# maxgillett/tinysplat

Measured on AMD Instinct MI355X. Metric: Gaussians*pixels/s fwd+bwd, higher is better.
Workload: dtype f32; 1 GPU; 1000000 random Gaussians, SH degree 3, 1920x1080, fwd+bwd (RGB), BASELINE configs[2]; max_per_tile=614, parallelism=single GPU, tile_lists=16x16 (gsplat's) (auto), gaussian_order=as generated (i.i.d.)

## Files before the change

### include/tinysplat_hip.h

```cpp
#ifndef TINYSPLAT_HIP_H
#define TINYSPLAT_HIP_H

#include <stdint.h>

#ifdef __cplusplus
extern "C" {
#endif

#define TS_ABI_VERSION 8

#define TS_E_BADARG (-1)
#define TS_E_DEGREE (-2)

#define TS_TILE 16
#define TS_SPLAT_RECORD_FLOATS 12
#define TS_PARTIAL_ROW_FLOATS 12

int ts_abi_version(void);

typedef struct ts_camera {
    float fx, fy, cx, cy;
    int32_t img_width, img_height;
    int32_t tile_bounds_x, tile_bounds_y;
    int32_t tile_row0, tile_rows;
    float glob_scale;
    float clip_thresh;
    int32_t wide_tiles;
    int32_t hints;
} ts_camera;
#define TS_HINT_BALANCED_WALK 1
#define TS_HINT_COOP_SPLIT (1 << 20)
#define TS_CAM_LIST_SEGMENTS(s) (((s) & 15) << 8)
#define TS_CAM_WHOLE_TILES(w16) (((w16) & 15) << 12)
#define TS_CAM_COOP_TILES(c16) (((c16) & 15) << 16)
int64_t ts_final_floats(const ts_camera* cam_host, int32_t channels);
int32_t ts_cut_tiles(const ts_camera* cam_host, int32_t* band, int32_t* whole);
int32_t ts_num_tiles(const ts_camera* cam_host);


#define TS_PROJECT_LOG_SCALES 1
#define TS_PROJECT_RAW_QUATS 2

int ts_project_fwd(int32_t n, const float* means3d, const float* scales, const float* quats,
                   const float* viewmat, const float* projmat, const ts_camera* cam_host,
                   int32_t flags, float* xys, float* depths, int32_t* radii, float* conics,
                   int32_t* num_tiles_hit, float* cov3d, void* stream);

int ts_project_bwd(int32_t n, const float* means3d, const float* scales, const float* quats,
                   const float* viewmat, const float* projmat, const ts_camera* cam_host,
                   int32_t flags, const int32_t* radii, const float* v_xy, const float* v_depth,
                   const float* v_conic, const float* v_cov3d,
                   float* v_means3d, float* v_scales, float* v_quats, void* stream);


int ts_sh_fwd(int32_t n, int32_t degrees_to_use, int32_t num_bases, const float* viewdirs,
              const float* coeffs, float* colors, void* stream);

int ts_sh_bwd(int32_t n, int32_t degrees_to_use, int32_t num_bases, const float* viewdirs,
              const float* v_colors, float* v_coeffs, void* stream);

int ts_sh_colors_fwd(int32_t n, int32_t degrees_to_use, int32_t num_bases, const float* means3d,
                     const float* origin, const float* colors_dc, const float* colors_rest,
                     float* colors, uint8_t* clamp_mask, const int32_t* live, void* stream);
int ts_sh_colors_bwd(int32_t n, int32_t degrees_to_use, int32_t num_bases, const float* means3d,
                     const float* origin, const uint8_t* clamp_mask, const float* v_colors,
                     float* v_colors_dc, float* v_colors_rest, void* stream);
int ts_colors_pack_fwd(int32_t n, int32_t degrees_to_use, int32_t num_bases, const float* means3d,
                       const float* origin, const float* colors_dc, const float* colors_rest,
                       uint8_t* clamp_mask, const int32_t* live, int32_t channels, int32_t flags,
                       const float* xys, const int32_t* radii, const float* conics, const float* opacity,
                       const int32_t* cum_tiles_hit, const ts_camera* cam_host, const float* depths,
                       float* splats, void* stream);


int64_t ts_scan_ws_ints(int32_t n);
int ts_scan_tiles(int32_t n, const int32_t* num_tiles_hit, int32_t* cum_tiles_hit,
                  int32_t* scan_ws, int32_t* total_out, void* stream);

int64_t ts_bin_ws_ints(int32_t n, int32_t num_tiles);

int ts_bin_count(int32_t n, const float* xys, const int32_t* radii, const float* splats,
                 const ts_camera* cam_host, int32_t* bin_ws, void* stream);

int ts_tile_offsets(int32_t n, int32_t num_tiles, int32_t* bin_ws, int32_t* tile_bins,
                    const int32_t* cum_tiles_hit, int64_t capacity, void* stream);
int ts_tile_offsets_stats(int32_t n, int32_t num_tiles, int32_t* bin_ws, int32_t* tile_bins,
                          const int32_t* cum_tiles_hit, int64_t capacity, int32_t* longest_list, void* stream);

int ts_bin_scatter(int32_t n, const float* xys, const int32_t* radii, const float* splats,
                   const ts_camera* cam_host, const int32_t* bin_ws, int32_t* bucket_ids, int32_t* scratch,
                   void* stream);

int ts_sort_tiles(int32_t num_tiles, const int32_t* tile_bins, const float* depths,
                  const int32_t* bucket_ids, int32_t* gaussian_ids_sorted, int32_t* sort_ws,
                  int32_t* zeroed_counter, void* stream);
int ts_sort_tiles_above(int32_t num_tiles, const int32_t* tile_bins, const float* depths,
                        const int32_t* bucket_ids, int32_t* gaussian_ids_sorted, int32_t* sort_ws,
                        int32_t* zeroed_counter, void* stream);

int32_t ts_bin_group_form(int32_t n);
int ts_bin_count_groups(int32_t n, const float* xys, const int32_t* radii, const float* splats,
                        const ts_camera* cam_host, int32_t* bin_ws, void* stream);
int ts_group_offsets(int32_t n, int32_t num_tiles, int32_t* bin_ws, int32_t* tile_bins,
                     const int32_t* cum_tiles_hit, int64_t capacity, int32_t* longest_list, void* stream);
int ts_bin_scatter_groups(int32_t n, const float* xys, const int32_t* radii, const float* splats,
                          const ts_camera* cam_host, int32_t* bin_ws, int32_t* tile_bins, int32_t* bucket_ids,
                          int32_t* scratch, void* stream);
int32_t ts_bin_one_walk_form(int32_t n, int32_t num_tiles);
int32_t ts_bin_stage_capacity(void);
int ts_bin_emit_groups(int32_t n, const float* xys, const int32_t* radii, const float* splats,
                       const ts_camera* cam_host, const int32_t* cum_tiles_hit, int64_t capacity, int32_t* bin_ws,
                       int32_t* scratch, void* stream);
int ts_emit_offsets(int32_t n, int32_t num_tiles, int32_t* bin_ws, int32_t* tile_bins,
                    const int32_t* cum_tiles_hit, int64_t capacity, int32_t* longest_list, void* stream);
int ts_bin_gather_groups(int32_t n, int32_t num_tiles, int32_t* bin_ws, int32_t* tile_bins, int32_t* bucket_ids,
                         const int32_t* scratch, void* stream);
int ts_sort_tiles_stats(int32_t num_tiles, const int32_t* tile_bins, const float* depths,
                        const int32_t* bucket_ids, int32_t* gaussian_ids_sorted, int32_t* sort_ws,
                        int32_t* zeroed_counter, int32_t n, const int32_t* bin_ws, int32_t* longest_list,
                        void* stream);
int ts_sort_tiles_above_stats(int32_t num_tiles, const int32_t* tile_bins, const float* depths,
                              const int32_t* bucket_ids, int32_t* gaussian_ids_sorted, int32_t n,
                              const int32_t* bin_ws, int32_t* longest_list, void* stream);

#define TS_RASTER_LOGIT_OPACITY 1

int ts_pack_splats(int32_t n, int32_t channels, int32_t flags, const float* xys, const int32_t* radii,
                   const float* conics, const float* colors, const float* opacity,
                   const int32_t* cum_tiles_hit, const ts_camera* cam_host, const float* depths,
                   float* splats, void* stream);
// ... 375 lines not shown
```

### tinysplat_amd/_lib.py

```python
from __future__ import annotations

import ctypes
import os
from ctypes import POINTER, c_double, c_float, c_int32, c_int64, c_void_p
from pathlib import Path

LIB_PATH = Path(os.environ["TS_LIB_PATH"]) if os.environ.get("TS_LIB_PATH") else \
    Path(__file__).resolve().parent / "csrc" / "libtinysplat_hip.so"
ABI_VERSION = 8
HINT_BALANCED_WALK = 1
HINT_COOP_SPLIT = 1 << 20
RASTER_LOGIT_OPACITY = 1
RASTER_CLAMP_RGB = 2
RASTER_SPLIT_BLOCKS = 4
RASTER_NARROW_WAVES = 8
FRAME_TIGHT = 1
FRAME_SPLIT = 2
FRAME_NARROW_WAVES = 8
FRAME_STRIPE = 16
FRAME_DIRECT_SCATTER = 32
FRAME_PLANES = 64
FRAME_SEPARATE_SORT = 128
FRAME_LIST_STATS = 256
FRAME_SURVIVORS = 512
# ... 30 lines not shown
                    "view34", "projview", "origin", "background",
                    "xys", "depths", "conics", "colors", "splats",
                    "radii", "num_tiles_hit", "cum_tiles_hit", "sh_mask",
                    "scan_ws", "bin_ws", "tile_bins", "total_host")]
                + [("num_intersects", c_int64), ("capacity", c_int64)]
                + [(name, c_void_p) for name in (
                    "bucket_ids", "gaussian_ids_sorted", "out_img", "final_Ts", "final_index", "clamp_mask",
                    "v_out_img", "partials", "row_flags",
                    "v_xy", "v_conic", "v_colors", "v_depth", "v_opacity",
                    "v_means", "v_scales", "v_quats", "v_colors_dc", "v_colors_rest",
                    "out_depth", "v_out_depth", "survivors")])


_FRAME = POINTER(TsFrame)


class TsAdam(ctypes.Structure):
    _fields_ = [("exp_avg", c_void_p * 6), ("exp_avg_sq", c_void_p * 6), ("lr", c_float * 6), ("step", c_int32 * 6),
                ("beta1", c_float), ("beta2", c_float), ("eps", c_float)]


_ADAM = POINTER(TsAdam)

MAX_RANKS = 16


class TsStripes(ctypes.Structure):
    _fields_ = [("num", c_int32), ("row", c_int32 * (MAX_RANKS + 1))]


_STRIPES = POINTER(TsStripes)


class TsRankStep(ctypes.Structure):
    _fields_ = [("stripes", TsStripes), ("group_base", c_int32 * (MAX_RANKS + 1)), ("gid_base", c_int32),
                ("send_rows", c_int32), ("recv_rows", c_int32), ("route_ws", c_void_p), ("counts", c_void_p),
                ("send", c_void_p), ("recv", c_void_p), ("grad_rows", c_void_p), ("back", c_void_p)]


_RANK = POINTER(TsRankStep)

ENTRY_PROBE = ctypes.CFUNCTYPE(None, ctypes.c_char_p, c_int32, c_void_p)

SIGNATURES = {
    "ts_abi_version": (c_int32, []),
    "ts_project_fwd": (c_int32, [c_int32, _P, _P, _P, _P, _P, _CAM, c_int32, _P, _P, _P, _P, _P, _P, _P]),
    "ts_project_bwd": (c_int32, [c_int32, _P, _P, _P, _P, _P, _CAM, c_int32, _P, _P, _P, _P, _P, _P, _P, _P, _P]),
    "ts_sh_fwd": (c_int32, [c_int32, c_int32, c_int32, _P, _P, _P, _P]),
    "ts_sh_bwd": (c_int32, [c_int32, c_int32, c_int32, _P, _P, _P, _P]),
    "ts_sh_colors_fwd": (c_int32, [c_int32, c_int32, c_int32, _P, _P, _P, _P, _P, _P, _P, _P]),
    "ts_sh_colors_bwd": (c_int32, [c_int32, c_int32, c_int32, _P, _P, _P, _P, _P, _P, _P]),
    "ts_scan_ws_ints": (c_int64, [c_int32]),
    "ts_scan_tiles": (c_int32, [c_int32, _P, _P, _P, _P, _P]),
    "ts_bin_ws_ints": (c_int64, [c_int32, c_int32]),
    "ts_bin_count": (c_int32, [c_int32, _P, _P, _P, _CAM, _P, _P]),
    "ts_tile_offsets": (c_int32, [c_int32, c_int32, _P, _P, _P, c_int64, _P]),
    "ts_tile_offsets_stats": (c_int32, [c_int32, c_int32, _P, _P, _P, c_int64, _P, _P]),
    "ts_bin_scatter": (c_int32, [c_int32, _P, _P, _P, _CAM, _P, _P, _P, _P]),
    "ts_sort_tiles": (c_int32, [c_int32, _P, _P, _P, _P, _P, _P, _P]),
    "ts_sort_tiles_above": (c_int32, [c_int32, _P, _P, _P, _P, _P, _P, _P]),
    "ts_bin_group_form": (c_int32, [c_int32]),
    "ts_bin_count_groups": (c_int32, [c_int32, _P, _P, _P, _CAM, _P, _P]),
    "ts_group_offsets": (c_int32, [c_int32, c_int32, _P, _P, _P, c_int64, _P, _P]),
    "ts_bin_scatter_groups": (c_int32, [c_int32, _P, _P, _P, _CAM, _P, _P, _P, _P, _P]),
    "ts_bin_one_walk_form": (c_int32, [c_int32, c_int32]),
    "ts_bin_stage_capacity": (c_int32, []),
    "ts_bin_emit_groups": (c_int32, [c_int32, _P, _P, _P, _CAM, _P, c_int64, _P, _P, _P]),
    "ts_emit_offsets": (c_int32, [c_int32, c_int32, _P, _P, _P, c_int64, _P, _P]),
    "ts_bin_gather_groups": (c_int32, [c_int32, c_int32, _P, _P, _P, _P, _P]),
    "ts_sort_tiles_stats": (c_int32, [c_int32, _P, _P, _P, _P, _P, _P, c_int32, _P, _P, _P]),
    "ts_sort_tiles_above_stats": (c_int32, [c_int32, _P, _P, _P, _P, c_int32, _P, _P, _P]),
    "ts_num_tiles": (c_int32, [_CAM]),
    "ts_final_floats": (c_int64, [_CAM, c_int32]),
    "ts_cut_tiles": (c_int32, [_CAM, _P, _P]),
    "ts_colors_pack_fwd": (c_int32, [c_int32, c_int32, c_int32, _P, _P, _P, _P, _P, _P, c_int32, c_int32,
                                     _P, _P, _P, _P, _P, _CAM, _P, _P, _P]),
    "ts_pack_splats": (c_int32, [c_int32, c_int32, c_int32, _P, _P, _P, _P, _P, _P, _CAM, _P, _P, _P]),
    "ts_raster_fwd": (c_int32, [c_int32, c_int32, _CAM, _P, _P, _P, _P, _P, _P, _P, _P, _P]),
    "ts_raster_bwd": (c_int32, [c_int32, c_int32, c_int64, _CAM, _P, _P, _P, _P, _P, _P, _P, _P, _P, _P, _P, _P]),
    "ts_raster_fwd_planes": (c_int32, [c_int32, c_int32, _CAM, _P, _P, _P, _P, _P, _P, _P, _P, _P, _P]),
    "ts_raster_fwd_sort": (c_int32, [c_int32, c_int32, _CAM, _P, _P, _P, _P, _P, _P, _P, _P, _P, _P, _P, _P]),
    "ts_raster_bwd_planes": (c_int32, [c_int32, c_int32, c_int64, _CAM, _P, _P, _P, _P, _P, _P, _P, _P, c_int32,
                                       _P, _P, _P, _P, _P]),
    "ts_bench_stream_read": (c_int32, [_P, c_int64, _P, _P]),
    "ts_bench_gather48": (c_int32, [_P, _P, c_int64, _P, _P]),
    "ts_photometric_ws_floats": (c_int64, [c_int32, c_int32]),
    "ts_photometric_loss": (c_int32, [c_int32, c_int32, _P, _P, c_float, c_float, _P, _P, _P]),
    "ts_photometric_loss_rgbd": (c_int32, [c_int32, c_int32, c_int32, _P, _P, _P, c_float, c_float, c_float, _P, _P, _P]),
    "ts_photometric_loss_planes": (c_int32, [c_int32, c_int32, _P, _P, _P, _P, c_float, c_float, c_float, _P, _P, _P,
                                             _P]),
    "ts_photometric_loss_reduce": (c_int32, [c_int32, c_int32, c_float, c_float, c_float, _P, _P, _P]),
    "ts_adam_step": (c_int32, [c_int32, _P, _P, _P, _P, _P, _P, _P, c_float, c_float, c_float, _P]),
    "ts_sh_colors_bwd_adam": (c_int32, [c_int32, c_int32, c_int32, _P, _P, _P, _P, _P, _P, _ADAM, _P]),
    "ts_project_bwd_adam": (c_int32, [c_int32, _P, _P, _P, _P, _P, _CAM, c_int32, _P, _P, _P, _P, _P, _P, _ADAM, _P]),
    "ts_frame_bwd_params_adam": (c_int32, [_FRAME, _ADAM, _P]),
    "ts_grad_accum": (c_int32, [c_int32, _P, _P, _P]),
    "ts_densify_classify": (c_int32, [c_int32, _P, _P, _P, POINTER(TsDensifyPolicy), _P, _P]),
    "ts_densify_ws_ints": (c_int64, [c_int32]),
    "ts_densify_plan": (c_int32, [c_int32, _P, _P, _P, _P, _P]),
    "ts_gather_rows": (c_int32, [c_int32, _P, _P, _P, c_int32, c_int32, _P, _P]),
    "ts_split_fixup": (c_int32, [c_int32, _P, _P, _P, _P, _P, _P, _P, _P]),
    "ts_ply_row_floats": (c_int32, [c_int32]),
    "ts_ply_pack_rows": (c_int32, [c_int32, c_int32, _P, _P, _P, _P, _P, _P, _P, _P]),
    "ts_ply_unpack_rows": (c_int32, [c_int32, c_int32, _P, _P, _P, _P, _P, _P, _P, _P]),
    "ts_reduce_partials": (c_int32, [c_int32, c_int32, c_int32, _P, _P, _P, _P, _P, _P, _P, _P, _P, _P, _P, _P]),
    "ts_route_ws_ints": (c_int64, [c_int32, c_int32]),
# ... 134 lines not shown
```

### tinysplat_amd/csrc/binning.hip

```cpp
#include <hip/hip_runtime.h>

#include "../../include/tinysplat_hip.h"
#include "host_util.h"
#include "pack.h"
#include "splat_math.h"

namespace {

constexpr int kThreads = 256;
constexpr int kScanItems = 4;
constexpr int kScanBlock = kThreads * kScanItems;

__device__ __forceinline__ int wave_inclusive_scan(int v) {
    const int lane = threadIdx.x & 63;
#pragma unroll
    for (int d = 1; d < 64; d <<= 1) {
        const int u = __shfl_up(v, d, 64);
        if (lane >= d) v += u;
    }
    return v;
}

template <int WAVES = 4>
__device__ __forceinline__ int block_inclusive_scan(int v, int* total) {
    __shared__ int wave_sums[WAVES];
    const int lane = threadIdx.x & 63, wave = threadIdx.x >> 6;
    int inc = wave_inclusive_scan(v);
    if (lane == 63) wave_sums[wave] = inc;
    __syncthreads();
    int add = 0, tot = 0;
#pragma unroll
    for (int w = 0; w < WAVES; ++w) {
        const int s = wave_sums[w];
        if (w < wave) add += s;
        tot += s;
    }
    *total = tot;
    __syncthreads();
    return inc + add;
}

__global__ __launch_bounds__(kThreads) void scan_local_kernel(int n, const int* __restrict__ in,
                                                              int* __restrict__ out,
                                                              int* __restrict__ block_sums,
                                                              int* __restrict__ total_out) {
    const int base = blockIdx.x * kScanBlock + threadIdx.x * kScanItems;
    int v[kScanItems];
    int sum = 0;
#pragma unroll
    for (int k = 0; k < kScanItems; ++k) {
        v[k] = (base + k < n) ? in[base + k] : 0;
        sum += v[k];
        v[k] = sum;
    }
    int total;
    const int inc = block_inclusive_scan(sum, &total);
    const int excl = inc - sum;
#pragma unroll
    for (int k = 0; k < kScanItems; ++k)
        if (base + k < n) {
            out[base + k] = v[k] + excl;
            if (total_out && gridDim.x == 1 && base + k == n - 1)
                __hip_atomic_store(total_out, v[k] + excl, __ATOMIC_RELEASE, __HIP_MEMORY_SCOPE_SYSTEM);
        }
    if (threadIdx.x == 0) block_sums[blockIdx.x] = total;
}

__global__ __launch_bounds__(kThreads) void scan_add_kernel(int n, int* __restrict__ out,
                                                            const int* __restrict__ block_sums,
                                                            int* __restrict__ total_out) {
    __shared__ int red[kThreads / 64];
    int part = 0;
    for (int j = threadIdx.x; j < (int)blockIdx.x; j += kThreads) part += block_sums[j];
#pragma unroll
    for (int d = 32; d >= 1; d >>= 1) part += __shfl_xor(part, d, 64);
    if ((threadIdx.x & 63) == 0) red[threadIdx.x >> 6] = part;
    __syncthreads();
    int add = 0;
#pragma unroll
    for (int w = 0; w < kThreads / 64; ++w) add += red[w];
    const int base = blockIdx.x * kScanBlock + threadIdx.x * kScanItems;
#pragma unroll
    for (int k = 0; k < kScanItems; ++k)
        if (base + k < n) {
            const int v = out[base + k] + add;
            if (blockIdx.x != 0) out[base + k] = v;
            if (total_out && base + k == n - 1)
                __hip_atomic_store(total_out, v, __ATOMIC_RELEASE, __HIP_MEMORY_SCOPE_SYSTEM);
        }
}

#ifndef TS_BIN_THREADS
#define TS_BIN_THREADS 1024
#endif
constexpr int kBinThreads = TS_BIN_THREADS;
#ifndef TS_BIN_CHUNK
#define TS_BIN_CHUNK 4096
#endif
constexpr int kBinChunkMin = TS_BIN_CHUNK;
constexpr int kBinMaxChunks = 512;
constexpr int kBinWindowMax = 36864;
constexpr int kBinTargetBlocks = 1;

__host__ __device__ inline int bin_num_chunks(int n) {
    int per = n / 192;
    per = per < 1024 ? 1024 : (per > kBinChunkMin ? kBinChunkMin : per);
    int b = (n + per - 1) / per;
    if (b < 1) b = 1;
    if (b > kBinMaxChunks) b = kBinMaxChunks;
    return b;
}

inline int bin_window_tiles(int n, int num_tiles) {
    const int chunks = bin_num_chunks(n);
    int nwin = (kBinTargetBlocks + chunks - 1) / chunks;
    const int max_win = (num_tiles + 255) / 256;
    if (nwin > max_win) nwin = max_win;
    if (nwin < 1) nwin = 1;
    int window = (num_tiles + nwin - 1) / nwin;
    window = (window + 63) & ~63;
    if (window > kBinWindowMax) window = kBinWindowMax;
    return window;
}

using ts::TightTest;

#ifndef TS_BIN_PRE
#define TS_BIN_PRE 2
#endif
constexpr int kBinPre = TS_BIN_PRE;
template <typename Emit>
__device__ __forceinline__ void walk_chunk(int g0, int g1, const float* __restrict__ xys,
                                           const int* __restrict__ radii,
                                           const float4* __restrict__ splats, const ts_camera& cam,
                                           Emit emit) {
    const int ws = cam.wide_tiles ? 1 : 0;
    const int tbx = (cam.tile_bounds_x + ws) >> ws;
    const bool tight_lists = splats != nullptr;
    for (int base = g0 + threadIdx.x; base < g1; base += kBinPre * kBinThreads) {
        int r[kBinPre];
        float2 xy[kBinPre];
        float4 q0[kBinPre], q1[kBinPre];
// ... 1031 lines not shown
    const int* __restrict__ tile_bins, const float* __restrict__ depths,
    const int* __restrict__ bucket_ids, int* __restrict__ ids_sorted,
    const int* __restrict__ large_count, const int* __restrict__ large_list) {
    __shared__ unsigned long long lds_large[kLargeLdsU64];
    const int count = *large_count;
    for (int q = blockIdx.x; q < count; q += gridDim.x) {
        const int2 range = reinterpret_cast<const int2*>(tile_bins)[large_list[q]];
        const int n = range.y - range.x;
        if (n <= kSortCap) continue;
        __syncthreads();
        sort_tile_sample(bucket_ids + range.x, depths, ids_sorted + range.x, n, lds_large);
    }
}

__global__ __launch_bounds__(kThreads) void sort_tiles_above_kernel(
    const int* __restrict__ tile_bins, const float* __restrict__ depths,
    const int* __restrict__ bucket_ids, int* __restrict__ ids_sorted, const ListStats stats) {
    __shared__ unsigned long long lds_u64[kLargeLdsU64 > kSortCap / 2 ? kLargeLdsU64 : kSortCap / 2];
    if (stats.group_max && blockIdx.x == 0) store_longest(stats);
    const int2 range = reinterpret_cast<const int2*>(tile_bins)[blockIdx.x];
    const int n = range.y - range.x;
    if (n <= kWaveSortMax) return;
    if (n <= kSortCap) sort_bucket_block(bucket_ids + range.x, depths, ids_sorted + range.x, n, lds_u64);
    else sort_tile_sample(bucket_ids + range.x, depths, ids_sorted + range.x, n, lds_u64);
}

__global__ __launch_bounds__(kThreads) void pack_splats_kernel(int n, const ts::PackArgs a,
                                                              const float* __restrict__ colors) {
    const int i = blockIdx.x * kThreads + threadIdx.x;
    if (i >= n) return;
    if (a.radii[i] <= 0) return;
    float c0, c1, c2, c3 = 0.0f;
    if (a.channels == 4 && a.depths == nullptr) {
        const float4 c = reinterpret_cast<const float4*>(colors)[i];
        c0 = c.x; c1 = c.y; c2 = c.z; c3 = c.w;
    } else {
        c0 = colors[3 * i]; c1 = colors[3 * i + 1]; c2 = colors[3 * i + 2];
        if (a.channels == 4) c3 = a.depths[i];
    }
    ts::pack_one(a, i, c0, c1, c2, c3);
}

}

extern "C" {

int32_t ts_num_tiles(const ts_camera* cam) {
    if (!cam) return 0;
    const int tbx = cam->wide_tiles ? (cam->tile_bounds_x + 1) / 2 : cam->tile_bounds_x;
    return cam->tile_rows * tbx;
}

int64_t ts_scan_ws_ints(int32_t n) {
    return n <= 0 ? 1 : (int64_t)((n + kScanBlock - 1) / kScanBlock);
}

int ts_scan_tiles(int32_t n, const int32_t* num_tiles_hit, int32_t* cum_tiles_hit,
                  int32_t* scan_ws, int32_t* total_out, void* stream) {
    if (n < 0) return TS_E_BADARG;
    if (n == 0) return 0;
    if (!num_tiles_hit || !cum_tiles_hit || !scan_ws) return TS_E_BADARG;
    hipStream_t s = (hipStream_t)stream;
    const int nb = (n + kScanBlock - 1) / kScanBlock;
    hipLaunchKernelGGL(scan_local_kernel, dim3(nb), dim3(kThreads), 0, s, n, num_tiles_hit,
                       cum_tiles_hit, scan_ws, total_out);
    if (nb > 1)
        hipLaunchKernelGGL(scan_add_kernel, dim3(nb), dim3(kThreads), 0, s, n, cum_tiles_hit, scan_ws,
                           total_out);
    return launch_status();
}

int64_t ts_bin_ws_ints(int32_t n, int32_t num_tiles) { return bin_geometry(n, num_tiles).spare + 1; }

int ts_bin_count(int32_t n, const float* xys, const int32_t* radii, const float* splats,
                 const ts_camera* cam, int32_t* bin_ws, void* stream) {
    if (n < 0 || !cam || !bin_ws) return TS_E_BADARG;
    const int nt = ts_num_tiles(cam);
    if (nt <= 0) return 0;
    if (n > 0 && (!xys || !radii)) return TS_E_BADARG;
    const BinGeometry g = bin_geometry(n, nt);
    const int window = bin_window_tiles(n, nt);
    const int windows = (nt + window - 1) / window;
    const size_t lds = (size_t)window * sizeof(int);
    if (lds > 64 * 1024)
        (void)hipFuncSetAttribute(reinterpret_cast<const void*>(&bin_count_kernel),
                                  hipFuncAttributeMaxDynamicSharedMemorySize, (int)lds);
    hipLaunchKernelGGL(bin_count_kernel, dim3(g.chunks, windows), dim3(kBinThreads), lds,
                       (hipStream_t)stream, n, g.chunk, xys, radii,
                       reinterpret_cast<const float4*>(splats), *cam, nt, window, bin_ws);
    return launch_status();
}

int ts_tile_offsets(int32_t n, int32_t num_tiles, int32_t* bin_ws, int32_t* tile_bins,
                    const int32_t* cum_tiles_hit, int64_t capacity, void* stream) {
    return ts_tile_offsets_stats(n, num_tiles, bin_ws, tile_bins, cum_tiles_hit, capacity, nullptr, stream);
}

int ts_tile_offsets_stats(int32_t n, int32_t num_tiles, int32_t* bin_ws, int32_t* tile_bins,
                          const int32_t* cum_tiles_hit, int64_t capacity, int32_t* longest_list, void* stream) {
    if (n < 0 || num_tiles < 0) return TS_E_BADARG;
    if (num_tiles == 0) return 0;
    if (!bin_ws || !tile_bins) return TS_E_BADARG;
    const BinGeometry g = bin_geometry(n, num_tiles);
    int* tile_total = bin_ws + g.tile_start;
    const int per_group = (g.chunks + kScanGroups - 1) / kScanGroups;
    hipStream_t s = (hipStream_t)stream;
    hipLaunchKernelGGL(column_scan_kernel, dim3((num_tiles + kColTiles - 1) / kColTiles),
                       dim3(kColTiles * kScanGroups), 0, s, num_tiles, g.chunks, per_group, bin_ws, tile_total, true);
    hipLaunchKernelGGL(tile_offsets_kernel, dim3(1), dim3(kOffsetsThreads), 0, s, num_tiles, tile_total,
                       tile_bins, bin_ws + g.spare,
                       (cum_tiles_hit && n > 0) ? cum_tiles_hit + (n - 1) : nullptr, (long long)capacity, longest_list);
    return launch_status();
}

int32_t ts_bin_group_form(int32_t n) { return two_hop(n) ? 1 : 0; }

int ts_bin_count_groups(int32_t n, const float* xys, const int32_t* radii, const float* splats,
                        const ts_camera* cam, int32_t* bin_ws, void* stream) {
    if (!cam || !bin_ws || !xys || !radii || !two_hop(n)) return TS_E_BADARG;
    const int nt = ts_num_tiles(cam);
    if (nt <= 0) return 0;
// ... 221 lines not shown
```

### tinysplat_amd/csrc/frame.hip

```cpp
#include <hip/hip_runtime.h>

#include <atomic>
#include <cstdlib>
#if !defined(TS_NO_ROCTX) && __has_include(<rocprofiler-sdk-roctx/roctx.h>)
#include <rocprofiler-sdk-roctx/roctx.h>
#define TS_HAVE_ROCTX 1
#else
#define TS_HAVE_ROCTX 0
#endif

#include "../../include/tinysplat_hip.h"
#include "raster_survivors.h"

struct TsRange {
#if TS_HAVE_ROCTX
    explicit TsRange(const char* name) { roctxRangePush(name); }
    ~TsRange() { roctxRangePop(); }
#else
    explicit TsRange(const char*) {}
#endif
};

static std::atomic<ts_entry_probe> g_probe{nullptr};
static std::atomic<void*> g_probe_user{nullptr};
// ... 47 lines not shown
    return ((f->cam.hints >> 8) & 15) > 1 && !f->cam.wide_tiles && !(f->flags & TS_FRAME_NARROW_WAVES);
}
inline int bwd_split(const ts_frame* f) {
    return ((f->flags & TS_FRAME_SPLIT) && !segmented(f)) ? TS_RASTER_SPLIT_BLOCKS : 0;
}
inline int small_n_fused() {
    static const int v = [] {
        const char* e = getenv("TS_SMALL_N_FUSED");
        return e ? atoi(e) : 262144;
    }();
    return v;
}
inline bool survivors(const ts_frame* f) {
    return (f->flags & TS_FRAME_SURVIVORS) && f->survivors && f->final_Ts && f->num_intersects > 0 &&
           f->cam.wide_tiles == 0 &&
           !(f->flags & (TS_FRAME_SPLIT | TS_FRAME_NARROW_WAVES | TS_FRAME_SEPARATE_SORT));
}
enum class ListForm { direct, matrix, group, one_walk };
inline ListForm list_form(const ts_frame* f) {
    if ((f->flags & TS_FRAME_DIRECT_SCATTER) || !ts_bin_group_form(f->n)) return ListForm::direct;
    if (!(f->flags & TS_FRAME_GROUP_COUNTS)) return ListForm::matrix;
    if ((f->flags & TS_FRAME_ONE_WALK) && !(f->cam.hints & TS_HINT_BALANCED_WALK) &&
        ts_bin_one_walk_form(f->n, num_tiles(f)))
        return ListForm::one_walk;
    return ListForm::group;
}
inline const float* tight_records(const ts_frame* f) { return (f->flags & TS_FRAME_TIGHT) ? f->splats : nullptr; }
inline int32_t* longest_word(const ts_frame* f) {
    if ((f->flags & TS_FRAME_LIST_STATS) && f->total_host) {
        int32_t* dev = mapped_pointer(f->total_host);
        if (dev) return dev + 1;
    }
    return nullptr;
}
inline int raster_flags(const ts_frame* f) {
    return TS_RASTER_CLAMP_RGB | ((f->flags & TS_FRAME_SPLIT) ? TS_RASTER_SPLIT_BLOCKS : 0) |
           ((f->flags & TS_FRAME_NARROW_WAVES) ? TS_RASTER_NARROW_WAVES : 0);
}
}

extern "C" {

int32_t ts_frame_struct_bytes(void) { return (int32_t)sizeof(ts_frame); }

int ts_set_entry_probe(ts_entry_probe fn, void* user) {
    g_probe_user.store(user, std::memory_order_relaxed);
    g_probe.store(fn, std::memory_order_release);
    return 0;
}

int ts_frame_fwd_project(const ts_frame* f, void* stream) {
    TsRange range_("ts_frame_fwd_project");
    if (bad(f)) return TS_E_BADARG;
    TS_TRY(TS_ENTRY("ts_project_fwd",
                    ts_project_fwd(f->n, f->means, f->scales, f->quats, f->view34, f->projview, &f->cam, 3, f->xys,
                                   f->depths, f->radii, f->conics, f->num_tiles_hit, nullptr, stream)));
    int32_t* total_dev = f->total_host ? mapped_pointer(f->total_host) : nullptr;
    TS_TRY(TS_ENTRY("ts_scan_tiles",
                    ts_scan_tiles(f->n, f->num_tiles_hit, f->cum_tiles_hit, f->scan_ws, total_dev, stream)));
    if (f->n > 0 && f->total_host && !total_dev) {
        const hipError_t e = hipMemcpyAsync(f->total_host, f->cum_tiles_hit + (f->n - 1), sizeof(int32_t),
                                            hipMemcpyDeviceToHost, (hipStream_t)stream);
        if (e != hipSuccess) return (int)e;
    }
    return 0;
}

int ts_frame_fwd_prepare(const ts_frame* f, void* stream) {
    TsRange range_("ts_frame_fwd_prepare");
    if (bad(f)) return TS_E_BADARG;
    TS_TRY(TS_ENTRY("ts_colors_pack_fwd",
                    ts_colors_pack_fwd(f->n, f->sh_degree, f->num_bases, f->means, f->origin, f->colors_dc,
                                       f->num_bases > 1 ? f->colors_rest : nullptr, f->sh_mask,
                                       (f->flags & TS_FRAME_STRIPE) ? f->num_tiles_hit : nullptr, f->channels,
                                       TS_RASTER_LOGIT_OPACITY, f->xys, f->radii, f->conics, f->opacities,
                                       f->cum_tiles_hit, &f->cam, f->channels == 4 ? f->depths : nullptr, f->splats,
                                       stream)));
    const float* tight = tight_records(f);
    switch (list_form(f)) {
    case ListForm::one_walk:
        return 0;
    case ListForm::group:
        TS_TRY(TS_ENTRY("ts_bin_count",
                        ts_bin_count_groups(f->n, f->xys, f->radii, tight, &f->cam, f->bin_ws, stream)));
        return TS_ENTRY("ts_tile_offsets",
                        ts_group_offsets(f->n, num_tiles(f), f->bin_ws, f->tile_bins, f->cum_tiles_hit, f->capacity,
                                         longest_word(f), stream));
    case ListForm::matrix:
    case ListForm::direct:
        TS_TRY(TS_ENTRY("ts_bin_count", ts_bin_count(f->n, f->xys, f->radii, tight, &f->cam, f->bin_ws, stream)));
        return TS_ENTRY("ts_tile_offsets",
                        ts_tile_offsets_stats(f->n, num_tiles(f), f->bin_ws, f->tile_bins, f->cum_tiles_hit,
                                              f->capacity, longest_word(f), stream));
    }
    return TS_E_BADARG;
}

int ts_frame_fwd_composite(const ts_frame* f, void* stream) {
    TsRange range_("ts_frame_fwd_composite");
    if (bad(f) || f->num_intersects < 0) return TS_E_BADARG;
    const bool planes = (f->flags & TS_FRAME_PLANES) != 0;
    if (planes && (f->channels != 4 || !f->out_depth)) return TS_E_BADARG;
    const bool fused_sort = f->num_intersects > 0 && f->cam.wide_tiles == 0 &&
                            !(f->flags & (TS_FRAME_NARROW_WAVES | TS_FRAME_SEPARATE_SORT));
    const ListForm form = list_form(f);
    const float* tight = tight_records(f);
    const bool listed = f->num_intersects > 0;
    int32_t* scratch = f->gaussian_ids_sorted;
    switch (form) {
    case ListForm::one_walk:
        TS_TRY(TS_ENTRY("ts_bin_scatter",
                        ts_bin_emit_groups(f->n, f->xys, f->radii, tight, &f->cam, f->cum_tiles_hit, f->capacity,
// ... 235 lines not shown
```

### tinysplat_amd/csrc/project.hip

```cpp
#include <hip/hip_runtime.h>

#include "../../include/tinysplat_hip.h"
#include "host_util.h"
#include "pack.h"
#include "splat_math.h"
#include "adam_math.h"

namespace {

constexpr int kThreads = 256;
#ifndef TS_SH_THREADS_FWD
#define TS_SH_THREADS_FWD 128
#endif
#ifndef TS_SH_THREADS_BWD
#define TS_SH_THREADS_BWD 256
#endif
typedef float f4v __attribute__((ext_vector_type(4)));
__device__ __forceinline__ void store4(float4* p, float a, float b, float c, float d) {
    f4v v = {a, b, c, d};
    __builtin_nontemporal_store(v, reinterpret_cast<f4v*>(p));
}
constexpr int kShThreadsFwd = TS_SH_THREADS_FWD, kShThreadsBwd = TS_SH_THREADS_BWD;
__device__ __forceinline__ float4 load4_stream(const float4* p) {
    const f4v v = __builtin_nontemporal_load(reinterpret_cast<const f4v*>(p));
    return make_float4(v.x, v.y, v.z, v.w);
}

#include "project_inputs.h"

__global__ __launch_bounds__(kThreads) void project_fwd_kernel(
    int n, const float* __restrict__ means3d, const float* __restrict__ scales,
    const float* __restrict__ quats, const float* __restrict__ viewmat,
    const float* __restrict__ projmat, const ts_camera cam, const int flags,
    float* __restrict__ xys, float* __restrict__ depths, int* __restrict__ radii,
    float* __restrict__ conics, int* __restrict__ num_tiles_hit, float* __restrict__ cov3d) {
    const int i = blockIdx.x * kThreads + threadIdx.x;
    if (i >= n) return;
    const ts::Cam C = load_cam(viewmat, projmat, cam);
    const float m[3] = {means3d[3 * i], means3d[3 * i + 1], means3d[3 * i + 2]};
    float s[3] = {scales[3 * i], scales[3 * i + 1], scales[3 * i + 2]};
    const float4 qv = reinterpret_cast<const float4*>(quats)[i];
    float q[4] = {qv.x, qv.y, qv.z, qv.w};
    prep_inputs(flags, s, q, nullptr);
    ts::ProjOut o;
    ts::project_one(C, m, s, q, o);
    reinterpret_cast<float2*>(xys)[i] = make_float2(o.x, o.y);
    depths[i] = o.depth;
    radii[i] = o.radius;
    conics[3 * i] = o.conic[0]; conics[3 * i + 1] = o.conic[1]; conics[3 * i + 2] = o.conic[2];
    num_tiles_hit[i] = o.tiles;
    if (cov3d) {
        float2* c3 = reinterpret_cast<float2*>(cov3d) + 3 * (size_t)i;
        c3[0] = make_float2(o.cov3d[0], o.cov3d[1]);
        c3[1] = make_float2(o.cov3d[2], o.cov3d[3]);
        c3[2] = make_float2(o.cov3d[4], o.cov3d[5]);
    }
}

struct ProjAdam {
    float *means, *scales, *quats, *opacities;
    const float* v_opacity;
    float *m_means, *v_means, *m_scales, *v_scales, *m_quats, *v_quats, *m_opac, *v_opac;
    ts::AdamCoef c_means, c_scales, c_quats, c_opac;
};
template <bool ADAM>
__global__ __launch_bounds__(kThreads) void project_bwd_kernel(
    int n, const float* __restrict__ means3d, const float* __restrict__ scales,
    const float* __restrict__ quats, const float* __restrict__ viewmat,
    const float* __restrict__ projmat, const ts_camera cam, const int flags,
    const int* __restrict__ radii, const float* __restrict__ v_xy, const float* __restrict__ v_depth,
    const float* __restrict__ v_conic, const float* __restrict__ v_cov3d,
    float* __restrict__ v_means3d, float* __restrict__ v_scales, float* __restrict__ v_quats, const ProjAdam ad) {
    const int i = blockIdx.x * kThreads + threadIdx.x;
    if (i >= n) return;
    ts::ProjGrad g;
    for (int k = 0; k < 3; ++k) { g.v_mean[k] = 0.0f; g.v_scale[k] = 0.0f; }
    for (int k = 0; k < 4; ++k) g.v_quat[k] = 0.0f;
    float pm[3] = {0.f, 0.f, 0.f}, ps[3] = {0.f, 0.f, 0.f}, pq[4] = {0.f, 0.f, 0.f, 0.f};
    if (ADAM) {
        pm[0] = means3d[3 * i]; pm[1] = means3d[3 * i + 1]; pm[2] = means3d[3 * i + 2];
        ps[0] = scales[3 * i]; ps[1] = scales[3 * i + 1]; ps[2] = scales[3 * i + 2];
        const float4 qv = reinterpret_cast<const float4*>(quats)[i];
        pq[0] = qv.x; pq[1] = qv.y; pq[2] = qv.z; pq[3] = qv.w;
    }
    if (radii[i] > 0) {
        const ts::Cam C = load_cam(viewmat, projmat, cam);
        const float m[3] = {ADAM ? pm[0] : means3d[3 * i], ADAM ? pm[1] : means3d[3 * i + 1], ADAM ? pm[2] : means3d[3 * i + 2]};
        float s[3] = {ADAM ? ps[0] : scales[3 * i], ADAM ? ps[1] : scales[3 * i + 1], ADAM ? ps[2] : scales[3 * i + 2]};
        float4 qv;
        if (ADAM) qv = make_float4(pq[0], pq[1], pq[2], pq[3]);
        else qv = reinterpret_cast<const float4*>(quats)[i];
        float q[4] = {qv.x, qv.y, qv.z, qv.w};
        float inv_n = 1.0f;
        prep_inputs(flags, s, q, &inv_n);
        const float2 vxy = reinterpret_cast<const float2*>(v_xy)[i];
        const float vx[2] = {vxy.x, vxy.y};
        const float vc[3] = {v_conic[3 * i], v_conic[3 * i + 1], v_conic[3 * i + 2]};
        float vcov[6];
        if (v_cov3d) {
            for (int k = 0; k < 6; ++k) vcov[k] = v_cov3d[6 * (size_t)i + k];
        }
        ts::project_one_vjp(C, m, s, q, vx, v_depth ? v_depth[i] : 0.0f, vc, v_cov3d ? vcov : nullptr, g);
        if (flags & TS_PROJECT_LOG_SCALES) {
            g.v_scale[0] *= s[0]; g.v_scale[1] *= s[1]; g.v_scale[2] *= s[2];
        }
        if (flags & TS_PROJECT_RAW_QUATS) {
            const float dotp = q[0] * g.v_quat[0] + q[1] * g.v_quat[1] + q[2] * g.v_quat[2] +
                               q[3] * g.v_quat[3];
            for (int k = 0; k < 4; ++k) g.v_quat[k] = (g.v_quat[k] - q[k] * dotp) * inv_n;
// ... 310 lines not shown
#pragma unroll
    for (int u = 0; u < U; ++u) acc[u] = make_float4(0.f, 0.f, 0.f, 0.f);
    for (; i + (U - 1) * stride < n16; i += U * stride) {
        float4 v[U];
#pragma unroll
        for (int u = 0; u < U; ++u) {
            const f4v t = __builtin_nontemporal_load(reinterpret_cast<const f4v*>(src + i + u * stride));
            v[u] = make_float4(t.x, t.y, t.z, t.w);
        }
#pragma unroll
        for (int u = 0; u < U; ++u) {
            acc[u].x += v[u].x; acc[u].y += v[u].y; acc[u].z += v[u].z; acc[u].w += v[u].w;
        }
    }
    for (; i < n16; i += stride) {
        const float4 v0 = src[i];
        acc[0].x += v0.x; acc[0].y += v0.y; acc[0].z += v0.z; acc[0].w += v0.w;
    }
    float t = 0.f;
#pragma unroll
    for (int u = 0; u < U; ++u) t += (acc[u].x + acc[u].y) + (acc[u].z + acc[u].w);
    if (t == 123456.789f) sink[0] = t;
}

__global__ __launch_bounds__(kThreads) void gather48_kernel(const float4* __restrict__ records,
                                                            const int* __restrict__ ids, size_t m,
                                                            float* __restrict__ sink) {
    const size_t stride = (size_t)gridDim.x * kThreads;
    float4 a = make_float4(0.f, 0.f, 0.f, 0.f);
    for (size_t j = (size_t)blockIdx.x * kThreads + threadIdx.x; j < m; j += stride) {
        const size_t g = (size_t)ids[j];
        const float4 q0 = records[3 * g], q1 = records[3 * g + 1], q2 = records[3 * g + 2];
        a.x += q0.x + q1.x + q2.x; a.y += q0.y + q1.y + q2.y; a.z += q0.z + q1.z + q2.z; a.w += q0.w + q1.w + q2.w;
    }
    if ((a.x + a.y) + (a.z + a.w) == 123456.789f) sink[0] = a.x;
}

}

extern "C" {

int ts_abi_version(void) { return TS_ABI_VERSION; }

int ts_project_fwd(int32_t n, const float* means3d, const float* scales, const float* quats,
                   const float* viewmat, const float* projmat, const ts_camera* cam,
                   int32_t flags, float* xys, float* depths, int32_t* radii, float* conics,
                   int32_t* num_tiles_hit, float* cov3d, void* stream) {
    if (n < 0 || !cam) return TS_E_BADARG;
    if (n == 0) return 0;
    if (!means3d || !scales || !quats || !viewmat || !projmat || !xys || !depths || !radii ||
        !conics || !num_tiles_hit)
        return TS_E_BADARG;
    const int grid = (n + kThreads - 1) / kThreads;
    hipLaunchKernelGGL(project_fwd_kernel, dim3(grid), dim3(kThreads), 0, (hipStream_t)stream, n,
                       means3d, scales, quats, viewmat, projmat, *cam, (int)flags, xys, depths, radii,
                       conics, num_tiles_hit, cov3d);
    return launch_status();
}

int ts_project_bwd(int32_t n, const float* means3d, const float* scales, const float* quats,
                   const float* viewmat, const float* projmat, const ts_camera* cam,
                   int32_t flags, const int32_t* radii, const float* v_xy, const float* v_depth,
                   const float* v_conic, const float* v_cov3d, float* v_means3d, float* v_scales,
                   float* v_quats, void* stream) {
    if (n < 0 || !cam) return TS_E_BADARG;
    if (n == 0) return 0;
    if (!means3d || !scales || !quats || !viewmat || !projmat || !radii || !v_xy ||
        !v_conic || !v_means3d || !v_scales || !v_quats)
        return TS_E_BADARG;
    const int grid = (n + kThreads - 1) / kThreads;
    hipLaunchKernelGGL(project_bwd_kernel<false>, dim3(grid), dim3(kThreads), 0, (hipStream_t)stream, n,
                       means3d, scales, quats, viewmat, projmat, *cam, (int)flags, radii, v_xy, v_depth,
                       v_conic, v_cov3d, v_means3d, v_scales, v_quats, ProjAdam{});
    return launch_status();
}

static bool adam_group_ok(const ts_adam* a, int k) {
    return a->exp_avg[k] && a->exp_avg_sq[k] && a->step[k] >= 1;
}

int ts_project_bwd_adam(int32_t n, float* means3d, float* scales, float* quats, const float* viewmat,
                        const float* projmat, const ts_camera* cam, int32_t flags, const int32_t* radii,
                        const float* v_xy, const float* v_depth, const float* v_conic, float* opacities,
                        const float* v_opacity, const ts_adam* adam, void* stream) {
    if (n < 0 || !cam || !adam) return TS_E_BADARG;
    if (n == 0) return 0;
    if (!means3d || !scales || !quats || !viewmat || !projmat || !radii || !v_xy || !v_conic) return TS_E_BADARG;
    if (!adam_group_ok(adam, TS_ADAM_MEANS) || !adam_group_ok(adam, TS_ADAM_SCALES) || !adam_group_ok(adam, TS_ADAM_QUATS))
        return TS_E_BADARG;
    if (opacities && (!v_opacity || !adam_group_ok(adam, TS_ADAM_OPACITIES))) return TS_E_BADARG;
    ProjAdam ad{};
    ad.means = means3d; ad.scales = scales; ad.quats = quats; ad.opacities = opacities; ad.v_opacity = v_opacity;
    ad.m_means = adam->exp_avg[TS_ADAM_MEANS]; ad.v_means = adam->exp_avg_sq[TS_ADAM_MEANS];
    ad.m_scales = adam->exp_avg[TS_ADAM_SCALES]; ad.v_scales = adam->exp_avg_sq[TS_ADAM_SCALES];
    ad.m_quats = adam->exp_avg[TS_ADAM_QUATS]; ad.v_quats = adam->exp_avg_sq[TS_ADAM_QUATS];
    ad.m_opac = adam->exp_avg[TS_ADAM_OPACITIES]; ad.v_opac = adam->exp_avg_sq[TS_ADAM_OPACITIES];
    auto coef = [&](int k) { return ts::adam_coef(adam->lr[k], adam->step[k], adam->beta1, adam->beta2, adam->eps); };
    ad.c_means = coef(TS_ADAM_MEANS); ad.c_scales = coef(TS_ADAM_SCALES); ad.c_quats = coef(TS_ADAM_QUATS);
    if (opacities) ad.c_opac = coef(TS_ADAM_OPACITIES);
    const int grid = (n + kThreads - 1) / kThreads;
    hipLaunchKernelGGL(project_bwd_kernel<true>, dim3(grid), dim3(kThreads), 0, (hipStream_t)stream, n,
                       means3d, scales, quats, viewmat, projmat, *cam, (int)flags, radii, v_xy, v_depth,
                       v_conic, (const float*)nullptr, (float*)nullptr, (float*)nullptr, (float*)nullptr, ad);
    return launch_status();
}

static int sh_check(int32_t n, int32_t degree, int32_t num_bases) {
    if (n < 0) return TS_E_BADARG;
    if (num_bases != 1 && num_bases != 4 && num_bases != 9 && num_bases != 16 && num_bases != 25)
// ... 218 lines not shown
```

Before: 2070000 billion Gaussians*pixels/s.

## Fuse tile-count block scan into projection kernel and add a blocked scan-add pass

The projection forward kernel now also runs a per-workgroup inclusive scan of tiles hit and writes local prefix sums plus one block sum per workgroup. A new add kernel then reduces the preceding block sums and adds the offsets with vectorised int4 accesses. This replaces the separate scan-local pass over num_tiles_hit, removing one kernel launch and one read of the counts array. The cost is a larger block-sum workspace, because scan blocks shrink to 256, and a redundant prefix reduction of block sums inside every add block.

After: 2074000 billion Gaussians*pixels/s (median of 2 runs). Within noise of the previous version (+0.2%).

```diff
diff --git a/include/tinysplat_hip.h b/include/tinysplat_hip.h
--- a/include/tinysplat_hip.h
+++ b/include/tinysplat_hip.h
@@ -76,6 +76,11 @@
 int64_t ts_scan_ws_ints(int32_t n);
 int ts_scan_tiles(int32_t n, const int32_t* num_tiles_hit, int32_t* cum_tiles_hit,
                   int32_t* scan_ws, int32_t* total_out, void* stream);
+int ts_project_fwd_scan(int32_t n, const float* means3d, const float* scales, const float* quats,
+                        const float* viewmat, const float* projmat, const ts_camera* cam_host, int32_t flags,
+                        float* xys, float* depths, int32_t* radii, float* conics, int32_t* num_tiles_hit,
+                        float* cov3d, int32_t* cum_tiles_hit, int32_t* scan_ws, int32_t* total_out, void* stream);
+int ts_scan_tiles_add(int32_t n, int32_t* cum_tiles_hit, const int32_t* scan_ws, int32_t* total_out, void* stream);
 
 int64_t ts_bin_ws_ints(int32_t n, int32_t num_tiles);
 
diff --git a/tinysplat_amd/_lib.py b/tinysplat_amd/_lib.py
--- a/tinysplat_amd/_lib.py
+++ b/tinysplat_amd/_lib.py
@@ -106,6 +106,8 @@
     "ts_sh_colors_bwd": (c_int32, [c_int32, c_int32, c_int32, _P, _P, _P, _P, _P, _P, _P]),
     "ts_scan_ws_ints": (c_int64, [c_int32]),
     "ts_scan_tiles": (c_int32, [c_int32, _P, _P, _P, _P, _P]),
+    "ts_project_fwd_scan": (c_int32, [c_int32, _P, _P, _P, _P, _P, _CAM, c_int32, _P, _P, _P, _P, _P, _P, _P, _P, _P, _P]),
+    "ts_scan_tiles_add": (c_int32, [c_int32, _P, _P, _P, _P]),
     "ts_bin_ws_ints": (c_int64, [c_int32, c_int32]),
     "ts_bin_count": (c_int32, [c_int32, _P, _P, _P, _CAM, _P, _P]),
     "ts_tile_offsets": (c_int32, [c_int32, c_int32, _P, _P, _P, c_int64, _P]),
diff --git a/tinysplat_amd/csrc/binning.hip b/tinysplat_amd/csrc/binning.hip
--- a/tinysplat_amd/csrc/binning.hip
+++ b/tinysplat_amd/csrc/binning.hip
@@ -11,34 +11,7 @@
 constexpr int kScanItems = 4;
 constexpr int kScanBlock = kThreads * kScanItems;
 
-__device__ __forceinline__ int wave_inclusive_scan(int v) {
-    const int lane = threadIdx.x & 63;
-#pragma unroll
-    for (int d = 1; d < 64; d <<= 1) {
-        const int u = __shfl_up(v, d, 64);
-        if (lane >= d) v += u;
-    }
-    return v;
-}
-
-template <int WAVES = 4>
-__device__ __forceinline__ int block_inclusive_scan(int v, int* total) {
-    __shared__ int wave_sums[WAVES];
-    const int lane = threadIdx.x & 63, wave = threadIdx.x >> 6;
-    int inc = wave_inclusive_scan(v);
-    if (lane == 63) wave_sums[wave] = inc;
-    __syncthreads();
-    int add = 0, tot = 0;
-#pragma unroll
-    for (int w = 0; w < WAVES; ++w) {
-        const int s = wave_sums[w];
-        if (w < wave) add += s;
-        tot += s;
-    }
-    *total = tot;
-    __syncthreads();
-    return inc + add;
-}
+#include "block_scan.h"
 
 __global__ __launch_bounds__(kThreads) void scan_local_kernel(int n, const int* __restrict__ in,
                                                               int* __restrict__ out,
@@ -88,6 +61,81 @@
             if (total_out && base + k == n - 1)
                 __hip_atomic_store(total_out, v, __ATOMIC_RELEASE, __HIP_MEMORY_SCOPE_SYSTEM);
         }
+}
+
+constexpr int kAddSums = 16;
+constexpr int kAddRounds = kAddSums * kProjectScanBlock / kScanBlock;
+static_assert(kProjectScanBlock == 256 && kThreads / 64 * kProjectScanBlock == kScanBlock, "a wave of a round = one block");
+__global__ __launch_bounds__(kThreads) void scan_add_kernel_proj(int n, int* __restrict__ out,
+                                                                 const int* __restrict__ block_sums,
+                                                                 int* __restrict__ total_out) {
+    __shared__ int red[kThreads / 64];
+    __shared__ int own[kAddSums];
+    const int first = blockIdx.x * kAddSums;
+    const bool vec = (reinterpret_cast<uintptr_t>(out) & 15) == 0;
+    const int base0 = blockIdx.x * (kAddSums * kProjectScanBlock) + threadIdx.x * kScanItems;
+    int4 v[kAddRounds];
+#pragma unroll
+    for (int r = 0; r < kAddRounds; ++r) {
+        const int base = base0 + r * kScanBlock;
+        if (vec && base + kScanItems <= n) v[r] = *reinterpret_cast<const int4*>(out + base);
+    }
+    int part = 0;
+    if ((reinterpret_cast<uintptr_t>(block_sums) & 15) == 0) {
+        const int4* sums4 = reinterpret_cast<const int4*>(block_sums);
+        for (int j0 = 0; j0 < first / 4; j0 += 4 * kThreads) {
+            int4 q[4];
+#pragma unroll
+            for (int u = 0; u < 4; ++u) {
+                const int j = j0 + u * kThreads + threadIdx.x;
+                q[u] = j < first / 4 ? sums4[j] : make_int4(0, 0, 0, 0);
+            }
+#pragma unroll
+            for (int u = 0; u < 4; ++u) part += (q[u].x + q[u].y) + (q[u].z + q[u].w);
+        }
+    } else {
+        for (int j = threadIdx.x; j < first; j += kThreads) part += block_sums[j];
+    }
+#pragma unroll
+    for (int d = 32; d >= 1; d >>= 1) part += __shfl_xor(part, d, 64);
+    if ((threadIdx.x & 63) == 0) red[threadIdx.x >> 6] = part;
+    if (threadIdx.x < kAddSums) {
+        const long long last = (long long)(first + threadIdx.x + 1) * kProjectScanBlock - 1;
+        own[threadIdx.x] = last < n ? out[last] : 0;
+    }
+    __syncthreads();
+    int add = 0;
+#pragma unroll
+    for (int w = 0; w < kThreads / 64; ++w) add += red[w];
+#pragma unroll
+    for (int r = 0; r < kAddRounds; ++r) {
+        const int sub = r * (kThreads / 64) + (threadIdx.x >> 6);
+        if (r > 0) {
+#pragma unroll
+            for (int w = 0; w < kThreads / 64; ++w) add += own[(r - 1) * (kThreads / 64) + w];
+        }
+        int a = add;
+#pragma unroll
+        for (int w = 0; w < kThreads / 64 - 1; ++w)
+            if (w < (int)(threadIdx.x >> 6)) a += own[r * (kThreads / 64) + w];
+        const int base = base0 + r * kScanBlock;
+        const bool first_block = blockIdx.x == 0 && sub == 0;
+        if (vec && base + kScanItems <= n) {
+            v[r].x += a; v[r].y += a; v[r].z += a; v[r].w += a;
+            if (!first_block) *reinterpret_cast<int4*>(out + base) = v[r];
+            if (total_out && base + kScanItems == n)
+                __hip_atomic_store(total_out, v[r].w, __ATOMIC_RELEASE, __HIP_MEMORY_SCOPE_SYSTEM);
+        } else {
+#pragma unroll
+            for (int k = 0; k < kScanItems; ++k)
+                if (base + k < n) {
+                    const int e = out[base + k] + a;
+                    if (!first_block) out[base + k] = e;
+                    if (total_out && base + k == n - 1)
+                        __hip_atomic_store(total_out, e, __ATOMIC_RELEASE, __HIP_MEMORY_SCOPE_SYSTEM);
+                }
+        }
+    }
 }
 
 #ifndef TS_BIN_THREADS
@@ -1225,7 +1273,7 @@
 }
 
 int64_t ts_scan_ws_ints(int32_t n) {
-    return n <= 0 ? 1 : (int64_t)((n + kScanBlock - 1) / kScanBlock);
+    return n <= 0 ? 1 : (int64_t)((n + kProjectScanBlock - 1) / kProjectScanBlock);
 }
 
 int ts_scan_tiles(int32_t n, const int32_t* num_tiles_hit, int32_t* cum_tiles_hit,
@@ -1240,6 +1288,17 @@
     if (nb > 1)
         hipLaunchKernelGGL(scan_add_kernel, dim3(nb), dim3(kThreads), 0, s, n, cum_tiles_hit, scan_ws,
                            total_out);
+    return launch_status();
+}
+
+int ts_scan_tiles_add(int32_t n, int32_t* cum_tiles_hit, const int32_t* scan_ws, int32_t* total_out, void* stream) {
+    if (n < 0) return TS_E_BADARG;
+    if (n <= kProjectScanBlock) return 0;
+    if (!cum_tiles_hit || !scan_ws) return TS_E_BADARG;
+    const int num_sums = (n + kProjectScanBlock - 1) / kProjectScanBlock;
+    const int nb = (num_sums + kAddSums - 1) / kAddSums;
+    hipLaunchKernelGGL(scan_add_kernel_proj, dim3(nb), dim3(kThreads), 0, (hipStream_t)stream, n, cum_tiles_hit, scan_ws,
+                       total_out);
     return launch_status();
 }
 
diff --git a/tinysplat_amd/csrc/block_scan.h b/tinysplat_amd/csrc/block_scan.h
--- /dev/null
+++ b/tinysplat_amd/csrc/block_scan.h
@@ -0,0 +1,32 @@
+#pragma once
+
+constexpr int kProjectScanBlock = 256;
+
+__device__ __forceinline__ int wave_inclusive_scan(int v) {
+    const int lane = threadIdx.x & 63;
+#pragma unroll
+    for (int d = 1; d < 64; d <<= 1) {
+        const int u = __shfl_up(v, d, 64);
+        if (lane >= d) v += u;
+    }
+    return v;
+}
+
+template <int WAVES = 4>
+__device__ __forceinline__ int block_inclusive_scan(int v, int* total) {
+    __shared__ int wave_sums[WAVES];
+    const int lane = threadIdx.x & 63, wave = threadIdx.x >> 6;
+    int inc = wave_inclusive_scan(v);
+    if (lane == 63) wave_sums[wave] = inc;
+    __syncthreads();
+    int add = 0, tot = 0;
+#pragma unroll
+    for (int w = 0; w < WAVES; ++w) {
+        const int s = wave_sums[w];
+        if (w < wave) add += s;
+        tot += s;
+    }
+    *total = tot;
+    __syncthreads();
+    return inc + add;
+}
diff --git a/tinysplat_amd/csrc/frame.hip b/tinysplat_amd/csrc/frame.hip
--- a/tinysplat_amd/csrc/frame.hip
+++ b/tinysplat_amd/csrc/frame.hip
@@ -123,12 +123,12 @@
 int ts_frame_fwd_project(const ts_frame* f, void* stream) {
     TsRange range_("ts_frame_fwd_project");
     if (bad(f)) return TS_E_BADARG;
+    int32_t* total_dev = f->total_host ? mapped_pointer(f->total_host) : nullptr;
     TS_TRY(TS_ENTRY("ts_project_fwd",
-                    ts_project_fwd(f->n, f->means, f->scales, f->quats, f->view34, f->projview, &f->cam, 3, f->xys,
-                                   f->depths, f->radii, f->conics, f->num_tiles_hit, nullptr, stream)));
-    int32_t* total_dev = f->total_host ? mapped_pointer(f->total_host) : nullptr;
-    TS_TRY(TS_ENTRY("ts_scan_tiles",
-                    ts_scan_tiles(f->n, f->num_tiles_hit, f->cum_tiles_hit, f->scan_ws, total_dev, stream)));
+                    ts_project_fwd_scan(f->n, f->means, f->scales, f->quats, f->view34, f->projview, &f->cam, 3, f->xys,
+                                        f->depths, f->radii, f->conics, f->num_tiles_hit, nullptr, f->cum_tiles_hit,
+                                        f->scan_ws, total_dev, stream)));
+    TS_TRY(TS_ENTRY("ts_scan_tiles", ts_scan_tiles_add(f->n, f->cum_tiles_hit, f->scan_ws, total_dev, stream)));
     if (f->n > 0 && f->total_host && !total_dev) {
         const hipError_t e = hipMemcpyAsync(f->total_host, f->cum_tiles_hit + (f->n - 1), sizeof(int32_t),
                                             hipMemcpyDeviceToHost, (hipStream_t)stream);
diff --git a/tinysplat_amd/csrc/project.hip b/tinysplat_amd/csrc/project.hip
--- a/tinysplat_amd/csrc/project.hip
+++ b/tinysplat_amd/csrc/project.hip
@@ -28,33 +28,60 @@
 
 #include "project_inputs.h"
 
+#include "block_scan.h"
+static_assert(kThreads == kProjectScanBlock, "one block sum per projection workgroup");
+
+template <bool SCAN>
 __global__ __launch_bounds__(kThreads) void project_fwd_kernel(
     int n, const float* __restrict__ means3d, const float* __restrict__ scales,
     const float* __restrict__ quats, const float* __restrict__ viewmat,
     const float* __restrict__ projmat, const ts_camera cam, const int flags,
     float* __restrict__ xys, float* __restrict__ depths, int* __restrict__ radii,
-    float* __restrict__ conics, int* __restrict__ num_tiles_hit, float* __restrict__ cov3d) {
+    float* __restrict__ conics, int* __restrict__ num_tiles_hit, float* __restrict__ cov3d,
+    int* __restrict__ cum_local, int* __restrict__ block_sums, int* __restrict__ total_out) {
     const int i = blockIdx.x * kThreads + threadIdx.x;
-    if (i >= n) return;
-    const ts::Cam C = load_cam(viewmat, projmat, cam);
-    const float m[3] = {means3d[3 * i], means3d[3 * i + 1], means3d[3 * i + 2]};
-    float s[3] = {scales[3 * i], scales[3 * i + 1], scales[3 * i + 2]};
-    const float4 qv = reinterpret_cast<const float4*>(quats)[i];
-    float q[4] = {qv.x, qv.y, qv.z, qv.w};
-    prep_inputs(flags, s, q, nullptr);
-    ts::ProjOut o;
-    ts::project_one(C, m, s, q, o);
-    reinterpret_cast<float2*>(xys)[i] = make_float2(o.x, o.y);
-    depths[i] = o.depth;
-    radii[i] = o.radius;
-    conics[3 * i] = o.conic[0]; conics[3 * i + 1] = o.conic[1]; conics[3 * i + 2] = o.conic[2];
-    num_tiles_hit[i] = o.tiles;
-    if (cov3d) {
-        float2* c3 = reinterpret_cast<float2*>(cov3d) + 3 * (size_t)i;
-        c3[0] = make_float2(o.cov3d[0], o.cov3d[1]);
-        c3[1] = make_float2(o.cov3d[2], o.cov3d[3]);
-        c3[2] = make_float2(o.cov3d[4], o.cov3d[5]);
-    }
+    if (!SCAN && i >= n) return;
+    int tiles = 0;
+    if (i < n) {
+        const ts::Cam C = load_cam(viewmat, projmat, cam);
+        const float m[3] = {means3d[3 * i], means3d[3 * i + 1], means3d[3 * i + 2]};
+        float s[3] = {scales[3 * i], scales[3 * i + 1], scales[3 * i + 2]};
+        const float4 qv = reinterpret_cast<const float4*>(quats)[i];
+        float q[4] = {qv.x, qv.y, qv.z, qv.w};
+        prep_inputs(flags, s, q, nullptr);
+        ts::ProjOut o;
+        ts::project_one(C, m, s, q, o);
+        reinterpret_cast<float2*>(xys)[i] = make_float2(o.x, o.y);
+        depths[i] = o.depth;
+        radii[i] = o.radius;
+        conics[3 * i] = o.conic[0]; conics[3 * i + 1] = o.conic[1]; conics[3 * i + 2] = o.conic[2];
+        num_tiles_hit[i] = o.tiles;
+        if (cov3d) {
+            float2* c3 = reinterpret_cast<float2*>(cov3d) + 3 * (size_t)i;
+            c3[0] = make_float2(o.cov3d[0], o.cov3d[1]);
+            c3[1] = make_float2(o.cov3d[2], o.cov3d[3]);
+            c3[2] = make_float2(o.cov3d[4], o.cov3d[5]);
+        }
+        tiles = o.tiles;
+    }
+    if (!SCAN) return;
+    __shared__ int wave_sums[kThreads / 64];
+    int inc = wave_inclusive_scan(tiles);
+    if ((threadIdx.x & 63) == 63) wave_sums[threadIdx.x >> 6] = inc;
+    __syncthreads();
+    int total = 0;
+#pragma unroll
+    for (int w = 0; w < kThreads / 64; ++w) {
+        const int s = wave_sums[w];
+        if (w < (int)(threadIdx.x >> 6)) inc += s;
+        total += s;
+    }
+    if (i < n) {
+        cum_local[i] = inc;
+        if (total_out && gridDim.x == 1 && i == n - 1)
+            __hip_atomic_store(total_out, inc, __ATOMIC_RELEASE, __HIP_MEMORY_SCOPE_SYSTEM);
+    }
+    if (threadIdx.x == 0) block_sums[blockIdx.x] = total;
 }
 
 struct ProjAdam {
@@ -471,9 +498,25 @@
         !conics || !num_tiles_hit)
         return TS_E_BADARG;
     const int grid = (n + kThreads - 1) / kThreads;
-    hipLaunchKernelGGL(project_fwd_kernel, dim3(grid), dim3(kThreads), 0, (hipStream_t)stream, n,
+    hipLaunchKernelGGL(project_fwd_kernel<false>, dim3(grid), dim3(kThreads), 0, (hipStream_t)stream, n,
                        means3d, scales, quats, viewmat, projmat, *cam, (int)flags, xys, depths, radii,
-                       conics, num_tiles_hit, cov3d);
+                       conics, num_tiles_hit, cov3d, (int*)nullptr, (int*)nullptr, (int*)nullptr);
+    return launch_status();
+}
+
+int ts_project_fwd_scan(int32_t n, const float* means3d, const float* scales, const float* quats,
+                        const float* viewmat, const float* projmat, const ts_camera* cam, int32_t flags,
+                        float* xys, float* depths, int32_t* radii, float* conics, int32_t* num_tiles_hit,
+                        float* cov3d, int32_t* cum_tiles_hit, int32_t* scan_ws, int32_t* total_out, void* stream) {
+    if (n < 0 || !cam) return TS_E_BADARG;
+    if (n == 0) return 0;
+    if (!means3d || !scales || !quats || !viewmat || !projmat || !xys || !depths || !radii ||
+        !conics || !num_tiles_hit || !cum_tiles_hit || !scan_ws)
+        return TS_E_BADARG;
+    const int grid = (n + kThreads - 1) / kThreads;
+    hipLaunchKernelGGL(project_fwd_kernel<true>, dim3(grid), dim3(kThreads), 0, (hipStream_t)stream, n,
+                       means3d, scales, quats, viewmat, projmat, *cam, (int)flags, xys, depths, radii,
+                       conics, num_tiles_hit, cov3d, cum_tiles_hit, scan_ws, total_out);
     return launch_status();
 }
 
```
